# Kuntz-Lab/interactive-rate-tendons

Measured on AMD Instinct MI355X. Metric: FK+collision checks/sec (3-tendon, 256^3 voxel env), higher is better.
Workload: dtype f64

## Files before the change

interactive-rate-tendons_amd/csrc/sample_host.inc:

```
namespace {

int sample_box(tr_ctx *c, const double *lo, const double *hi, trk::SampleBox &box) {
  const int N = c->K.n_tendons, S = c->K.state_size;
  box = trk::SampleBox{};
  box.S = S;
  for (int d = 0; d < S; d++) {
    double a, b;
    if (lo && hi) { a = lo[d]; b = hi[d]; }
    else if (d < N) { a = 0.0; b = c->max_tension[(size_t)d]; }
    else if (c->K.enable_rotation && d == N) { a = -M_PI; b = M_PI; }
    else { a = 0.0; b = c->K.L; }
    if (!(b >= a) || !std::isfinite(a) || !std::isfinite(b)) return fail(c, TR_ERR_INVALID_ARG, "sampling bounds must be finite with hi >= lo");
    box.lo[d] = a; box.span[d] = b - a;
  }
  return TR_OK;
}

int ensure_sample_scratch(tr_ctx *c, int64_t batch, int64_t out_cap) {
  tr_ctx::Sampler &sm = c->samp;
  const size_t S = (size_t)c->K.state_size;
  int rc;
  if (!sm.d_ctr) {
    if ((rc = dev_alloc(c, &sm.d_ctr, 1))) return rc;
    HIP_TRY(c, hipHostMalloc((void **)&sm.h_ctr, sizeof(trk::SampleCounters), hipHostMallocDefault));
// ... 97 lines not shown
  return TR_OK;
}

}

extern "C" {

int tr_candidate_states_dev(tr_ctx *c, uint64_t seed, uint64_t first, int64_t count, const double *lo, const double *hi,
                            double *d_states, void *stream) {
  if (!c) return TR_ERR_INVALID_ARG;
  std::lock_guard<std::recursive_mutex> lock_(c->mu);
  if (count < 0 || (count > 0 && !d_states) || (!lo != !hi)) return fail(c, TR_ERR_INVALID_ARG, "bad argument");
  if (count == 0) return TR_OK;
  HIP_TRY(c, hipSetDevice(c->device));
  trk::SampleBox box;
  int rc;
  if ((rc = sample_box(c, lo, hi, box))) return rc;
  trk::launch_candidate_states(seed, first, count, box, d_states, (hipStream_t)stream);
  HIP_TRY(c, hipGetLastError());
  return TR_OK;
}

int tr_candidate_states(tr_ctx *c, uint64_t seed, uint64_t first, int64_t count, const double *lo, const double *hi, double *states) {
  if (!c) return TR_ERR_INVALID_ARG;
  std::lock_guard<std::recursive_mutex> lock_(c->mu);
  if (count < 0 || (count > 0 && !states) || (!lo != !hi)) return fail(c, TR_ERR_INVALID_ARG, "bad argument");
  if (count == 0) return TR_OK;
  HIP_TRY(c, hipSetDevice(c->device));
  int rc;
  const int S = c->K.state_size;
  const int64_t chunk = (int64_t)1 << 22;
  if ((rc = ensure_sample_scratch(c, std::min(count, chunk), c->samp.out_cap))) return rc;
  if ((rc = ensure_pipe(c))) return rc;
  hipStream_t s = c->pipe.s_comp;
  if ((rc = begin_dev_work(c, s))) return rc;
  trk::SampleBox box;
  if ((rc = sample_box(c, lo, hi, box))) return rc;
  for (int64_t off = 0; off < count; off += chunk) {
    const int64_t m = std::min(chunk, count - off);
    trk::launch_candidate_states(seed, first + (uint64_t)off, m, box, c->samp.states, s);
    HIP_TRY(c, hipGetLastError());
    HIP_TRY(c, hipMemcpyAsync(states + off * S, c->samp.states, (size_t)m * S * sizeof(double), hipMemcpyDeviceToHost, s));
    HIP_TRY(c, hipStreamSynchronize(s));
  }
  return note_dev_work(c, s);
}

static int validate_candidates_dev_impl(tr_ctx *c, uint64_t seed, uint64_t first, int64_t count, const double *lo, const double *hi,
                                        uint64_t *d_valid_bits, double *d_tips, uint8_t *d_flags, uint32_t *d_sig, void *stream) {
  if (!c) return TR_ERR_INVALID_ARG;
  std::lock_guard<std::recursive_mutex> lock_(c->mu);
  if (count < 0 || (count > 0 && !d_valid_bits) || (!lo != !hi)) return fail(c, TR_ERR_INVALID_ARG, "bad argument");
  if (count == 0) return TR_OK;
  if (first % 64) return fail(c, TR_ERR_INVALID_ARG, "first candidate must be a multiple of 64 (whole mask words)");
  HIP_TRY(c, hipSetDevice(c->device));
  hipStream_t s = (hipStream_t)stream;
  int rc;
  if ((rc = begin_dev_work(c, s))) return rc;
  trk::SampleBox box;
  if ((rc = sample_box(c, lo, hi, box))) return rc;
  const int S = c->K.state_size;
  const int64_t chunk = (int64_t)1 << 22;
  if ((rc = ensure_sample_scratch(c, std::min(count, chunk), c->samp.out_cap))) return rc;
  for (int64_t off = 0; off < count; off += chunk) {
    const int64_t m = std::min(chunk, count - off);
    trk::launch_candidate_states(seed, first + (uint64_t)off, m, box, c->samp.states, s);
    HIP_TRY(c, hipGetLastError());
// ... 97 lines not shown
  if (!c) return TR_ERR_INVALID_ARG;
  std::lock_guard<std::recursive_mutex> lock_(c->mu);
  if ((n_want > 0 && !d_states) || (!lo != !hi)) return fail(c, TR_ERR_INVALID_ARG, "bad argument");
  HIP_TRY(c, hipSetDevice(c->device));
  int rc;
  if ((rc = begin_dev_work(c, (hipStream_t)stream))) return rc;
  if ((rc = sample_valid_impl(c, seed, first_candidate, lo, hi, n_want, max_candidates, d_states, d_tips, d_index, n_accepted, n_tried,
                              (hipStream_t)stream))) return rc;
  return note_dev_work(c, (hipStream_t)stream);
}

int tr_sample_valid_vertices_sig_dev(tr_ctx *c, uint64_t seed, uint64_t first_candidate, const double *lo, const double *hi, int64_t n_want,
                                     int64_t max_candidates, double *d_states, double *d_tips, int64_t *d_index, uint32_t *d_sig,
                                     int64_t *n_accepted, int64_t *n_tried, void *stream) {
  if (!c) return TR_ERR_INVALID_ARG;
  std::lock_guard<std::recursive_mutex> lock_(c->mu);
  if ((n_want > 0 && (!d_states || !d_sig)) || (!lo != !hi)) return fail(c, TR_ERR_INVALID_ARG, "bad argument");
  HIP_TRY(c, hipSetDevice(c->device));
  int rc;
  if ((rc = begin_dev_work(c, (hipStream_t)stream))) return rc;
  if ((rc = sample_valid_impl(c, seed, first_candidate, lo, hi, n_want, max_candidates, d_states, d_tips, d_index, n_accepted, n_tried,
                              (hipStream_t)stream, d_sig))) return rc;
  return note_dev_work(c, (hipStream_t)stream);
}

int tr_sample_valid_vertices(tr_ctx *c, uint64_t seed, uint64_t first_candidate, const double *lo, const double *hi, int64_t n_want,
                             int64_t max_candidates, double *states, double *tips, int64_t *index, int64_t *n_accepted, int64_t *n_tried) {
  if (!c) return TR_ERR_INVALID_ARG;
  std::lock_guard<std::recursive_mutex> lock_(c->mu);
  if ((n_want > 0 && !states) || (!lo != !hi)) return fail(c, TR_ERR_INVALID_ARG, "bad argument");
  HIP_TRY(c, hipSetDevice(c->device));
  int rc;
  if ((rc = ensure_pipe(c))) return rc;
  hipStream_t s = c->pipe.s_comp;
  if ((rc = begin_dev_work(c, s))) return rc;
  int64_t have = 0;
  if ((rc = sample_valid_impl(c, seed, first_candidate, lo, hi, n_want, max_candidates, nullptr, nullptr, nullptr, &have, n_tried, s))) return rc;
  if (n_accepted) *n_accepted = have;
  if (have > 0) {
    const size_t S = (size_t)c->K.state_size;
    HIP_TRY(c, hipMemcpyAsync(states, c->samp.out_states, (size_t)have * S * sizeof(double), hipMemcpyDeviceToHost, s));
    if (tips) HIP_TRY(c, hipMemcpyAsync(tips, c->samp.out_tips, (size_t)have * 3 * sizeof(double), hipMemcpyDeviceToHost, s));
    if (index) HIP_TRY(c, hipMemcpyAsync(index, c->samp.out_index, (size_t)have * sizeof(int64_t), hipMemcpyDeviceToHost, s));
    HIP_TRY(c, hipStreamSynchronize(s));
  }
  return note_dev_work(c, s);
}

}
```

interactive-rate-tendons_amd/csrc/tendon_hip.hip:

```cpp
#include <hip/hip_runtime.h>
#include <sched.h>

#include <algorithm>
#include <cfloat>
#include <cmath>
#include <cstdio>
#include <cstdlib>
#include <cstring>
#include <functional>
#include <initializer_list>
#include <chrono>
#include <thread>
#include <ctime>
#include <limits>
#include <mutex>
#include <string>
#include <vector>

#include "../../include/tendon_hip.h"
#include "tr_types.hpp"
#include "fk_launch.hpp"
#include "fk_lin_launch.hpp"
#include "sweep_kernel.hpp"
#include "sphere_kernel.hpp"
#include "verdict_kernel.hpp"
#include "edge_kernel.hpp"
#include "edge_plan.hpp"
#include "routing_form.hpp"
#include "knn_kernel.hpp"
#include "cache_merge.hpp"
#include "env_kernel.hpp"
#include "sample.hpp"
#include "ik_kernel.hpp"
#include "fk_loaded_kernel.hpp"
#include "loaded_edge_kernel.hpp"
#include "loaded_roadmap_kernel.hpp"
#include "loaded_ik_kernel.hpp"
#include "loaded_sens_kernel.hpp"

void tr_dev_cache_trim();
struct tr_ctx;
namespace { void ik_release(tr_ctx *c); }
namespace { void shoot_release(tr_ctx *c); }
namespace { void ikl_release(tr_ctx *c); }

namespace {

std::string g_create_error;

struct Workspace {
  int64_t ld = 0;
  double *px = nullptr, *py = nullptr, *pz = nullptr, *acc = nullptr;
  double *Li = nullptr;
  double *homeLi = nullptr;
  int32_t *np = nullptr;
  uint8_t *conv = nullptr;
  int64_t st_cap = 0;
  double *states = nullptr;
  uint64_t *bits = nullptr;
  double *tips = nullptr;
  uint8_t *flags = nullptr;
// ... 106 lines not shown
  bool edge_lanes_fixed = false;
  bool edge_kernels_loaded = false;
  bool edge_queue = true;
  bool edge_queue_forced = false;
  int edge_queue_waves = 0;
  uint32_t edge_queue_last[4] = {0, 0, 0, 0};
  double edge_rate_seen = 0.0;
  bool edge_lane_guess_forced = false;
  double edge_lane_guess = 6.0;
  int64_t retract_sort_min = kRetractSortMin;
  bool rows_one_step = false;
  bool retract_wave_start = true;
  struct VerdictRing {
    static constexpr int kSlots = 16;
    trk::VerdictArgs *d_slots = nullptr, *h_slots = nullptr;
    hipEvent_t ev[kSlots];
    bool used[kSlots] = {};
    int next = 0;
  } vring;
  struct FusedRing {
    static constexpr int kSlots = 16;
    trk::FusedSweepArgs *d_slots = nullptr, *h_slots = nullptr;
    hipEvent_t ev[kSlots];
    bool used[kSlots] = {};
    int next = 0;
  } fused;
  struct KnnScratch { void *p[13] = {}; size_t cap[13] = {}; } knn;
  struct VoxStore { uint32_t *ids = nullptr; uint64_t *masks = nullptr; int64_t cap = 0, n = 0; } vstore;
  uint32_t *d_vids = nullptr; uint64_t *d_vmasks = nullptr; int32_t *d_vcounts = nullptr;
  uint64_t *d_vbits = nullptr;
  int64_t vox_cap = 0;
  int32_t *d_item_src = nullptr, *d_item_edge = nullptr; int64_t vox_items_cap = 0;
  struct Pipe {
    bool ready = false;
    int64_t chunk = 0;
    hipStream_t s_up = nullptr, s_comp = nullptr, s_down = nullptr;
    double *h_states[2] = {nullptr, nullptr}; double *h_tips[2] = {nullptr, nullptr};
    uint64_t *h_bits[2] = {nullptr, nullptr}; uint8_t *h_flags[2] = {nullptr, nullptr};
    hipEvent_t up[2], done[2], down[2];
  } pipe;
  hipEvent_t last_dev_ev = nullptr;
  bool last_dev_used = false;
  hipStream_t last_dev_stream = nullptr;
  struct Sampler {
    int64_t cap = 0;
    double *states = nullptr; uint64_t *bits = nullptr; double *tips = nullptr; uint32_t *wprefix = nullptr;
    uint32_t *wprefix2 = nullptr; int64_t wp2_cap = 0;
    trk::SampleCounters *d_ctr = nullptr, *h_ctr = nullptr;
    int64_t out_cap = 0;
    double *out_states = nullptr, *out_tips = nullptr; int64_t *out_index = nullptr;
    double rate_seen = 0.0;
    uint32_t *sig = nullptr; int64_t sig_cap = 0;
    int64_t *sig_index = nullptr; int64_t sig_index_cap = 0;
  } samp;
  void *h_stage = nullptr; size_t h_stage_cap = 0;
  struct IkDev {
    int64_t probs = 0, lanes = 0;
    double *xs = nullptr, *tips = nullptr;
    double *p = nullptr, *pn = nullptr, *f = nullptr, *J = nullptr, *des = nullptr;
    double *err2 = nullptr, *mu = nullptr, *nu = nullptr;
    int32_t *iters = nullptr, *calls = nullptr, *list[2] = {nullptr, nullptr};
    RoundCount count;
    double *io_s = nullptr, *io_3 = nullptr, *io_e = nullptr;
    int32_t *io_i = nullptr, *io_c = nullptr;
    DevOwner chunk, once;
  } ik;
  struct ShootDev {
    int64_t probs = 0, lanes = 0;
    double *xs = nullptr, *res = nullptr;
    double *p = nullptr, *pn = nullptr, *e = nullptr, *J = nullptr;
    double *err2 = nullptr, *mu = nullptr, *nu = nullptr;
    int32_t *iters = nullptr, *calls = nullptr, *list[2] = {nullptr, nullptr};
// ... 778 lines not shown
    }
  PolyK poly{};
  for (int j = 0; j < N; j++) {
    for (int i = 0; i < rb->n_a; i++) poly.C[j][i] = c->C[(size_t)j * rb->n_a + i];
    for (int i = 0; i < rb->n_m; i++) poly.D[j][i] = c->D[(size_t)j * rb->n_m + i];
    const int rdeg = poly_degree(&c->D[(size_t)j * rb->n_m], rb->n_m), tdeg = poly_degree(&c->C[(size_t)j * rb->n_a], rb->n_a);
    poly.home_kind[j] = (rdeg == 0 && tdeg == 0) ? 0 : ((rdeg == 0 && tdeg == 1) ? 1 : 2);
    const double d0 = poly.D[j][0], c1 = rb->n_a > 1 ? poly.C[j][1] : 0.0;
    poly.helix_scale[j] = std::sqrt(1 + d0 * d0 * c1 * c1);
  }

  auto bail = [&](const char *what) { std::string m = what; tr_destroy(c); return fail(nullptr, TR_ERR_HIP, m); };
  if (hipMalloc((void **)&c->d_poly, sizeof(PolyK)) != hipSuccess) return bail("hipMalloc(poly)");
  if (hipMemcpy(c->d_poly, &poly, sizeof(PolyK), hipMemcpyHostToDevice) != hipSuccess) return bail("hipMemcpy(poly)");
  if (hipMalloc((void **)&c->d_tgrid, c->t.size() * sizeof(double)) != hipSuccess ||
      hipMalloc((void **)&c->d_hl, hl.size() * sizeof(double)) != hipSuccess) return bail("hipMalloc(tgrid)");
  if (hipMemcpy(c->d_tgrid, c->t.data(), c->t.size() * sizeof(double), hipMemcpyHostToDevice) != hipSuccess ||
      hipMemcpy(c->d_hl, hl.data(), hl.size() * sizeof(double), hipMemcpyHostToDevice) != hipSuccess) return bail("hipMemcpy(tgrid)");
  if (hipMalloc((void **)&c->d_tab, tab.size() * sizeof(double)) != hipSuccess) return bail("hipMalloc(tab)");
  if (hipMemcpy(c->d_tab, tab.data(), tab.size() * sizeof(double), hipMemcpyHostToDevice) != hipSuccess) return bail("hipMemcpy(tab)");
  if (hipMalloc((void **)&c->d_steps, std::max<size_t>(1, c->steps.size()) * sizeof(StepK)) != hipSuccess) return bail("hipMalloc(steps)");
  if (!c->steps.empty() &&
      hipMemcpy(c->d_steps, c->steps.data(), c->steps.size() * sizeof(StepK), hipMemcpyHostToDevice) != hipSuccess) return bail("hipMemcpy(steps)");
  *out = c;
  return TR_OK;
}

void tr_destroy(tr_ctx *c) {
  if (!c) return;
  (void)hipSetDevice(c->device);
  (void)hipDeviceSynchronize();
  for (auto &v : c->events) for (auto &e : v) { (void)hipEventDestroy(e.a); (void)hipEventDestroy(e.b); }
  if (c->pipe.ready) {
    for (int b = 0; b < 2; b++) {
      (void)hipHostFree(c->pipe.h_states[b]); (void)hipHostFree(c->pipe.h_tips[b]); (void)hipHostFree(c->pipe.h_bits[b]); (void)hipHostFree(c->pipe.h_flags[b]);
      (void)hipEventDestroy(c->pipe.up[b]); (void)hipEventDestroy(c->pipe.done[b]); (void)hipEventDestroy(c->pipe.down[b]);
    }
    (void)hipStreamDestroy(c->pipe.s_up); (void)hipStreamDestroy(c->pipe.s_comp); (void)hipStreamDestroy(c->pipe.s_down);
  }
  Workspace &w = c->ws;
  void *ptrs[] = {c->d_tab, c->d_steps, c->d_poly, c->d_tgrid, c->d_hl, c->d_grid, c->d_near, w.homeLi, w.np, c->d_vids, c->d_vmasks, c->d_vcounts,
                  c->d_vbits, w.px, w.py, w.pz, w.acc, w.Li, w.conv,
                  w.states, w.bits, w.tips, w.flags, w.L, w.npts,
                  c->edge.lvl_states, c->edge.bits, c->edge.sample_edge, c->edge.sample_t, c->edge.open, c->edge.frontier,
                  c->edge.A, c->edge.B, c->edge.rel, c->edge.edge_ok, c->edge.nfk, c->edge.first_inv, c->edge.last_t, c->edge.nd, c->edge.cnt, c->edge.sig, c->edge.sig_np, c->edge.ix_states, c->edge.ix_idx, c->edge.open2, c->edge.lvl_states2, c->edge.q_remaining, c->edge.q_lvl_base, c->edge.q_lvl_cnt, c->edge.q_ctl, c->edge.q_args, c->d_envw[0], c->d_envw[1], c->d_sph_near, c->d_sph_tmp};
  for (void *p : ptrs) if (p) (void)hipFree(p);
  trk::merge_free(c->merge);
  if (c->fused.d_slots) { (void)hipFree(c->fused.d_slots); (void)hipHostFree(c->fused.h_slots); for (auto &e : c->fused.ev) (void)hipEventDestroy(e); }
  if (c->vring.d_slots) { (void)hipFree(c->vring.d_slots); (void)hipHostFree(c->vring.h_slots); for (auto &e : c->vring.ev) (void)hipEventDestroy(e); }
  if (c->last_dev_ev) (void)hipEventDestroy(c->last_dev_ev);
  {
    tr_ctx::Sampler &sm = c->samp;
    void *sp[] = {sm.states, sm.bits, sm.tips, sm.wprefix, sm.wprefix2, sm.d_ctr, sm.out_states, sm.out_tips, sm.out_index, sm.sig, sm.sig_index};
    for (void *q : sp) if (q) (void)hipFree(q);
    if (sm.h_ctr) (void)hipHostFree(sm.h_ctr);
  }
  if (c->d_item_src) (void)hipFree(c->d_item_src);
  if (c->d_item_edge) (void)hipFree(c->d_item_edge);
  for (void *q : c->knn.p) if (q) (void)hipFree(q);
  if (c->vstore.ids) (void)hipFree(c->vstore.ids);
  if (c->vstore.masks) (void)hipFree(c->vstore.masks);
  if (c->edge.q_hctl) (void)hipHostFree(c->edge.q_hctl);
  if (c->edge.q_hargs) (void)hipHostFree(c->edge.q_hargs);
  if (c->h_stage) (void)hipHostFree(c->h_stage);
  for (auto &ln : c->lane) {
    tr_ctx::RetractOrder &ro = ln.ro;
    void *lp[] = {ln.counters, ln.fb_list, ln.fb_count, ro.keys[0], ro.keys[1], ro.vals[0], ro.vals[1], ro.kbegin, ro.handoff};
    for (void *q : lp) if (q) (void)hipFree(q);
    if (ln.stream) (void)hipStreamDestroy(ln.stream);
    if (ln.hc) (void)hipHostFree(ln.hc);
    trk::merge_free(ro.ms);
// ... 349 lines not shown
  }
  (void)d_n_points;
  if ((rc = begin_dev_work(c, (hipStream_t)stream))) return rc;
  trk::SweepIn in{d_px, d_py, d_pz, nullptr, d_Li, d_converged, nullptr, c->ws.acc};
  if ((rc = launch_sweep(c, in, n, ld, check_voxels, d_valid_bits, d_flags, (hipStream_t)stream))) return rc;
  return note_dev_work(c, (hipStream_t)stream);
}

int tr_validate_shapes_retraction_dev(tr_ctx *c, int64_t n, int64_t ld, const double *d_px, const double *d_py,
                                      const double *d_pz, const int32_t *d_n_points, const double *d_Li,
                                      const double *d_home_Li, const uint8_t *d_converged, int check_voxels,
                                      uint64_t *d_valid_bits, uint8_t *d_flags, void *stream) {
  if (!c) return TR_ERR_INVALID_ARG;
  std::lock_guard<std::recursive_mutex> lock_(c->mu);
  if (!c->K.enable_retraction) return fail(c, TR_ERR_INVALID_ARG, "robot has no retraction: use tr_validate_shapes_dev");
  if (n < 0 || ld < n || (ld & 63)) return fail(c, TR_ERR_INVALID_ARG, "ld must be a multiple of 64 and >= n");
  if (n == 0) return TR_OK;
  if (!d_px || !d_py || !d_pz || !d_n_points || !d_Li || !d_home_Li || !d_converged || !d_valid_bits)
    return fail(c, TR_ERR_INVALID_ARG, "null device pointer");
  int rc;
  if (c->ws.ld < ld) {
    if (ld > c->max_chunk) return fail(c, TR_ERR_INVALID_ARG, "ld exceeds the workspace chunk size; call in smaller batches");
    if ((rc = ensure_workspace(c, ld))) return rc;
  }
  trk::SweepIn in{d_px, d_py, d_pz, d_n_points, d_Li, d_converged, d_home_Li, c->ws.acc};
  if ((rc = begin_dev_work(c, (hipStream_t)stream))) return rc;
  if ((rc = launch_sweep(c, in, n, ld, check_voxels, d_valid_bits, d_flags, (hipStream_t)stream))) return rc;
  return note_dev_work(c, (hipStream_t)stream);
}

}
namespace {
int validate_batch_dev_impl(tr_ctx *c, const double *d_states, int64_t n, uint64_t *d_valid_bits,
                            double *d_tips, uint8_t *d_flags, void *stream, uint32_t *d_sig = nullptr);
}
extern "C" {
int tr_validate_batch_dev(tr_ctx *c, const double *d_states, int64_t n, uint64_t *d_valid_bits,
                          double *d_tips, uint8_t *d_flags, void *stream) {
  if (!c) return TR_ERR_INVALID_ARG;
  std::lock_guard<std::recursive_mutex> lock_(c->mu);
  int rc;
  if ((rc = begin_dev_work(c, (hipStream_t)stream))) return rc;
  rc = validate_batch_dev_impl(c, d_states, n, d_valid_bits, d_tips, d_flags, stream);
  if (rc == TR_OK && n > 0) return note_dev_work(c, (hipStream_t)stream);
  return rc;
}
}
namespace {
int validate_batch_dev_impl(tr_ctx *c, const double *d_states, int64_t n, uint64_t *d_valid_bits,
                            double *d_tips, uint8_t *d_flags, void *stream, uint32_t *d_sig) {
  if (n < 0) return fail(c, TR_ERR_INVALID_ARG, "negative batch size");
  if (n == 0) return TR_OK;
  if (!d_states || !d_valid_bits) return fail(c, TR_ERR_INVALID_ARG, "null device pointer");
  if (!c->has_grid) return fail(c, TR_ERR_INVALID_ARG, "no obstacle grid set (tr_set_grid)");
  int rc;
  hipStream_t s = (hipStream_t)stream;
  const int S = c->K.state_size;
  const bool ret = c->K.enable_retraction;
  const int64_t sig_words = round_up(c->K.n_points, 16);
  if (d_sig && (c->fuse != 2 || ret || c->checker == TR_CHECKER_SPHERES)) return fail(c, TR_ERR_UNSUPPORTED, "signatures: backbone checker, no retraction, verdict-only schedule");
  if (c->fuse == 2) {
    const int64_t chunk = (int64_t)1 << 26;
    for (int64_t off = 0; off < n; off += chunk) {
      const int64_t m = std::min<int64_t>(chunk, n - off);
      if ((rc = launch_verdict(c, d_states + off * S, m, d_valid_bits + off / 64, d_tips ? d_tips + 3 * off : nullptr,
                               d_flags ? d_flags + off : nullptr, s, d_sig ? d_sig + off * sig_words : nullptr, d_sig ? sig_words : 0,
                               c->checker == TR_CHECKER_SPHERES))) return rc;
    }
    return TR_OK;
  }
  if ((rc = ensure_workspace(c, n))) return rc;
  Workspace &w = c->ws;
  for (int64_t off = 0; off < n; off += w.ld) {
    const int64_t m = std::min<int64_t>(w.ld, n - off);
    trk::FkOut out{w.px, w.py, w.pz, nullptr, nullptr, w.Li, d_tips ? d_tips + 3 * off : nullptr, w.conv,
                   ret ? w.np : nullptr, ret ? w.homeLi : nullptr};
    trk::SweepIn in{w.px, w.py, w.pz, ret ? w.np : nullptr, w.Li, w.conv, ret ? w.homeLi : nullptr, w.acc};
    if ((rc = launch_fk_sweep(c, d_states + off * S, m, w.ld, out, in, c->checker == TR_CHECKER_SPHERES ? 2 : 1, d_valid_bits + off / 64,
                              d_flags ? d_flags + off : nullptr, s))) return rc;
  }
  return TR_OK;
}
}
extern "C" {

namespace {
int ensure_pipe(tr_ctx *c) {
  tr_ctx::Pipe &p = c->pipe;
  if (p.ready) return TR_OK;
  int64_t CH = std::max<int64_t>(1 << 14, c->k1_round);
  if (const char *e = std::getenv("TENDON_HIP_PIPE_LOG2")) { const int v = std::atoi(e); if (v >= 12 && v <= 22) CH = (int64_t)1 << v; }
  const int S = c->K.state_size;
  HIP_TRY(c, hipStreamCreateWithFlags(&p.s_up, hipStreamNonBlocking));
  HIP_TRY(c, hipStreamCreateWithFlags(&p.s_comp, hipStreamNonBlocking));
  HIP_TRY(c, hipStreamCreateWithFlags(&p.s_down, hipStreamNonBlocking));
  for (int b = 0; b < 2; b++) {
    HIP_TRY(c, hipHostMalloc((void **)&p.h_states[b], (size_t)CH * S * sizeof(double), hipHostMallocDefault));
    HIP_TRY(c, hipHostMalloc((void **)&p.h_tips[b], (size_t)CH * 3 * sizeof(double), hipHostMallocDefault));
    HIP_TRY(c, hipHostMalloc((void **)&p.h_bits[b], (size_t)(CH / 64) * sizeof(uint64_t), hipHostMallocDefault));
    HIP_TRY(c, hipHostMalloc((void **)&p.h_flags[b], (size_t)CH, hipHostMallocDefault));
    HIP_TRY(c, hipEventCreateWithFlags(&p.up[b], hipEventDisableTiming));
    HIP_TRY(c, hipEventCreateWithFlags(&p.done[b], hipEventDisableTiming));
    HIP_TRY(c, hipEventCreateWithFlags(&p.down[b], hipEventDisableTiming));
  }
  p.chunk = CH;
  p.ready = true;
  return TR_OK;
}
}

int tr_validate_batch(tr_ctx *c, const double *states, int64_t n, uint64_t *valid_bits, double *tips, uint8_t *flags) {
  if (!c) return TR_ERR_INVALID_ARG;
  std::lock_guard<std::recursive_mutex> lock_(c->mu);
  if (n < 0 || (n > 0 && (!states || !valid_bits))) return fail(c, TR_ERR_INVALID_ARG, "bad argument");
  if (n == 0) return TR_OK;
  if (!c->has_grid) return fail(c, TR_ERR_INVALID_ARG, "no obstacle grid set (tr_set_grid)");
  HIP_TRY(c, hipSetDevice(c->device));
  int rc;
  if ((rc = ensure_pipe(c))) return rc;
  tr_ctx::Pipe &p = c->pipe;
  const int64_t CH = p.chunk;
  if (n <= kSmallBatch && n <= CH) {
    const int S = c->K.state_size;
    const bool verdict = c->fuse == 2;
    if ((rc = ensure_staging(c, n))) return rc;
    if (!verdict && (rc = ensure_workspace(c, n))) return rc;
    Workspace &w = c->ws;
    if ((rc = begin_dev_work(c, p.s_comp))) return rc;
    std::memcpy(p.h_states[0], states, (size_t)n * S * sizeof(double));
    HIP_TRY(c, hipMemcpyAsync(w.states, p.h_states[0], (size_t)n * S * sizeof(double), hipMemcpyHostToDevice, p.s_comp));
    if ((rc = validate_batch_dev_impl(c, w.states, n, w.bits, tips ? w.tips : nullptr, flags ? w.flags : nullptr, p.s_comp))) return rc;
    HIP_TRY(c, hipMemcpyAsync(p.h_bits[0], w.bits, (size_t)((n + 63) / 64) * sizeof(uint64_t), hipMemcpyDeviceToHost, p.s_comp));
    if (tips) HIP_TRY(c, hipMemcpyAsync(p.h_tips[0], w.tips, (size_t)n * 3 * sizeof(double), hipMemcpyDeviceToHost, p.s_comp));
    if (flags) HIP_TRY(c, hipMemcpyAsync(p.h_flags[0], w.flags, (size_t)n, hipMemcpyDeviceToHost, p.s_comp));
    HIP_TRY(c, hipStreamSynchronize(p.s_comp));
    c->last_dev_used = false;
    std::memcpy(valid_bits, p.h_bits[0], (size_t)((n + 63) / 64) * sizeof(uint64_t));
    if (tips) std::memcpy(tips, p.h_tips[0], (size_t)n * 3 * sizeof(double));
    if (flags) std::memcpy(flags, p.h_flags[0], (size_t)n);
    return TR_OK;
  }
  if ((rc = ensure_staging(c, std::min(n, 2 * CH)))) return rc;
  if (c->fuse != 2 && (rc = ensure_workspace(c, std::min(n, CH)))) return rc;
  HIP_TRY(c, hipDeviceSynchronize());
  Workspace &w = c->ws;
  const int S = c->K.state_size;
  const int64_t nchunks = (n + CH - 1) / CH;
  auto drain = [&](int64_t i) -> int {
    const int b = (int)(i & 1);
    const int64_t off = i * CH, m = std::min(CH, n - off);
    HIP_TRY(c, hipEventSynchronize(p.down[b]));
    std::memcpy(valid_bits + off / 64, p.h_bits[b], (size_t)((m + 63) / 64) * sizeof(uint64_t));
    if (tips) std::memcpy(tips + 3 * off, p.h_tips[b], (size_t)m * 3 * sizeof(double));
    if (flags) std::memcpy(flags + off, p.h_flags[b], (size_t)m);
    return TR_OK;
  };
  for (int64_t i = 0; i < nchunks; i++) {
    const int b = (int)(i & 1);
    const int64_t off = i * CH, m = std::min(CH, n - off);
    if (i >= 2 && (rc = drain(i - 2))) return rc;
    double *d_st = w.states + (size_t)b * CH * S;
    uint64_t *d_bits = w.bits + (size_t)b * (CH / 64);
    double *d_tips = w.tips + (size_t)b * CH * 3;
    uint8_t *d_flags = w.flags + (size_t)b * CH;
    std::memcpy(p.h_states[b], states + off * S, (size_t)m * S * sizeof(double));
    HIP_TRY(c, hipMemcpyAsync(d_st, p.h_states[b], (size_t)m * S * sizeof(double), hipMemcpyHostToDevice, p.s_up));
    HIP_TRY(c, hipEventRecord(p.up[b], p.s_up));
    HIP_TRY(c, hipStreamWaitEvent(p.s_comp, p.up[b], 0));
    if (i >= 2) HIP_TRY(c, hipStreamWaitEvent(p.s_comp, p.down[b], 0));
    if ((rc = validate_batch_dev_impl(c, d_st, m, d_bits, tips ? d_tips : nullptr, flags ? d_flags : nullptr, p.s_comp))) return rc;
    HIP_TRY(c, hipEventRecord(p.done[b], p.s_comp));
    HIP_TRY(c, hipStreamWaitEvent(p.s_down, p.done[b], 0));
    HIP_TRY(c, hipMemcpyAsync(p.h_bits[b], d_bits, (size_t)((m + 63) / 64) * sizeof(uint64_t), hipMemcpyDeviceToHost, p.s_down));
    if (tips) HIP_TRY(c, hipMemcpyAsync(p.h_tips[b], d_tips, (size_t)m * 3 * sizeof(double), hipMemcpyDeviceToHost, p.s_down));
    if (flags) HIP_TRY(c, hipMemcpyAsync(p.h_flags[b], d_flags, (size_t)m, hipMemcpyDeviceToHost, p.s_down));
    HIP_TRY(c, hipEventRecord(p.down[b], p.s_down));
  }
  for (int64_t i = std::max<int64_t>(0, nchunks - 2); i < nchunks; i++)
    if ((rc = drain(i))) return rc;
  return TR_OK;
}

int tr_check_cached_dev(tr_ctx *c, const uint32_t *d_ids, const uint64_t *d_masks, const int64_t *d_offsets,
                        int64_t n_items, uint64_t *d_hit_bits, void *stream) {
  if (!c) return TR_ERR_INVALID_ARG;
  std::lock_guard<std::recursive_mutex> lock_(c->mu);
  if (n_items < 0) return fail(c, TR_ERR_INVALID_ARG, "negative item count");
  if (n_items == 0) return TR_OK;
  if (!c->has_grid) return fail(c, TR_ERR_INVALID_ARG, "no obstacle grid set (tr_set_grid)");
  if (!d_ids || !d_masks || !d_offsets || !d_hit_bits) return fail(c, TR_ERR_INVALID_ARG, "null device pointer");
  hipStream_t s = (hipStream_t)stream;
  ProfScope ps(c, 2, s);
  const unsigned grid = (unsigned)((n_items + 3) / 4);
  HIP_TRY(c, hipMemsetAsync(d_hit_bits, 0, (size_t)((n_items + 63) / 64) * sizeof(uint64_t), s));
  hipLaunchKernelGGL(trk::cached_blocks_vs_grid, dim3(grid), dim3(64), 0, s, d_ids, d_masks, d_offsets, n_items,
                     c->d_grid, c->n_blocks, d_hit_bits);
  HIP_TRY(c, hipGetLastError());
  return TR_OK;
}

int tr_check_cached_subset_dev(tr_ctx *c, const uint32_t *d_ids, const uint64_t *d_masks, const int64_t *d_offsets,
                               int64_t n_items, const int32_t *d_list, int64_t n_list, uint8_t *d_hit, void *stream) {
  if (!c) return TR_ERR_INVALID_ARG;
  std::lock_guard<std::recursive_mutex> lock_(c->mu);
  if (n_items < 0 || n_list < 0) return fail(c, TR_ERR_INVALID_ARG, "negative count");
  if (n_list == 0) return TR_OK;
  if (!c->has_grid) return fail(c, TR_ERR_INVALID_ARG, "no obstacle grid set (tr_set_grid)");
  if (!d_ids || !d_masks || !d_offsets || !d_list || !d_hit) return fail(c, TR_ERR_INVALID_ARG, "null device pointer");
  hipStream_t s = (hipStream_t)stream;
  ProfScope ps(c, 2, s);
  hipLaunchKernelGGL(trk::cached_subset_vs_grid, dim3((unsigned)((n_list + 15) / 16)), dim3(256), 0, s, d_ids, d_masks, d_offsets,
                     d_list, n_list, n_items, c->d_grid, c->n_blocks, d_hit);
// ... 485 lines not shown
```

profiles/probe_host_pipe.py:

```python
#!/usr/bin/env python3
import importlib
import json
import os
import sys
import time

import numpy as np

ROOT = os.path.dirname(os.path.dirname(os.path.abspath(__file__)))
sys.path.insert(0, ROOT)


def main():
    import torch
    irt = importlib.import_module("interactive-rate-tendons_amd")
    W = irt.workloads
    robot = W.robot_config2()
    vox, _ = W.reach_environment(seed=7, n_spheres=64)
    n = 1 << 20
    states = W.random_states(robot, n, seed=3, tau_max=10.0)
    out = {}
    for log2 in (None, 14, 15, 16, 17, 18):
        if log2 is None:
            os.environ.pop("TENDON_HIP_PIPE_LOG2", None)
        else:
            os.environ["TENDON_HIP_PIPE_LOG2"] = str(log2)
        chk = irt.VoxelBackboneValidityChecker(robot, irt.VoxelEnvironment(), vox)
        eng = chk.engine
        for _ in range(2):
            eng.validate_batch(states)
        ts = []
        for _ in range(8):
            t0 = time.perf_counter()
            eng.validate_batch(states)
            ts.append(time.perf_counter() - t0)
        ts2 = []
        for _ in range(8):
            t0 = time.perf_counter()
            eng.validate_batch(states, want_tips=False, want_flags=False)
            ts2.append(time.perf_counter() - t0)
        d = torch.from_numpy(states).cuda()
        bits = torch.zeros(n // 64, dtype=torch.int64, device="cuda")
        tips = torch.zeros(n, 3, dtype=torch.float64, device="cuda")
        eng.validate_batch_dev(d, n, bits, tips)
        torch.cuda.synchronize()
        t0 = time.perf_counter()
# ... 17 lines not shown
```

Before: 137.6 million.

## Grade host pipeline chunk sizes and alternate compute across two lanes

Measured after the change: 137.8 million, median of 6. About the same (+0.1%).

```diff
diff --git a/interactive-rate-tendons_amd/csrc/pipe_schedule.hpp b/interactive-rate-tendons_amd/csrc/pipe_schedule.hpp
--- /dev/null
+++ b/interactive-rate-tendons_amd/csrc/pipe_schedule.hpp
@@ -0,0 +1,55 @@
+#pragma once
+#include <algorithm>
+#include <cstdint>
+#include <vector>
+
+namespace pipe_schedule {
+
+struct Chunk { int64_t offset, count; };
+
+constexpr int64_t kWave = 64;
+constexpr int64_t kGrade = 2;
+
+inline int64_t end_size(int64_t steady) {
+  const int64_t q = steady / kGrade / kWave * kWave;
+  return std::min(steady, std::max(q, kWave));
+}
+
+inline int64_t max_chunks(int64_t n, int64_t steady) {
+  int64_t ramp = 0;
+  for (int64_t s = end_size(steady); s < steady; s *= 2) ramp++;
+  return n / steady + 2 * ramp + 2;
+}
+inline std::vector<Chunk> graded(int64_t n, int64_t steady) {
+  std::vector<Chunk> out;
+  if (n <= 0 || steady < kWave) return out;
+  steady = steady / kWave * kWave;
+  const int64_t q = end_size(steady);
+  std::vector<int64_t> up, down;
+  for (int64_t s = q; s < steady; s *= 2) up.push_back(s);
+  down.assign(up.rbegin(), up.rend());
+  int64_t ramps = 0;
+  for (int64_t s : up) ramps += 2 * s;
+  std::vector<int64_t> counts;
+  if (n < ramps + steady) {
+    const int64_t k = (n + steady - 1) / steady;
+    const int64_t each = std::min(steady, ((n + k - 1) / k + kWave - 1) / kWave * kWave);
+    for (int64_t left = n; left > 0; left -= each) counts.push_back(std::min(each, left));
+  } else {
+    counts = up;
+    int64_t mid = n - ramps;
+    for (; mid >= steady; mid -= steady) counts.push_back(steady);
+    const int64_t odd = mid % kWave;
+    if (mid - odd > 0) counts.push_back(mid - odd);
+    counts.insert(counts.end(), down.begin(), down.end());
+    if (odd > 0) {
+      if (!down.empty() && counts.back() + odd <= steady) counts.back() += odd;
+      else counts.push_back(odd);
+    }
+  }
+  int64_t off = 0;
+  for (int64_t m : counts) { out.push_back(Chunk{off, m}); off += m; }
+  return out;
+}
+
+}
diff --git a/interactive-rate-tendons_amd/csrc/sample_host.inc b/interactive-rate-tendons_amd/csrc/sample_host.inc
--- a/interactive-rate-tendons_amd/csrc/sample_host.inc
+++ b/interactive-rate-tendons_amd/csrc/sample_host.inc
@@ -153,7 +153,7 @@
   const int64_t chunk = (int64_t)1 << 22;
   if ((rc = ensure_sample_scratch(c, std::min(count, chunk), c->samp.out_cap))) return rc;
   if ((rc = ensure_pipe(c))) return rc;
-  hipStream_t s = c->pipe.s_comp;
+  hipStream_t s = c->pipe.s_comp[0];
   if ((rc = begin_dev_work(c, s))) return rc;
   trk::SampleBox box;
   if ((rc = sample_box(c, lo, hi, box))) return rc;
@@ -317,7 +317,7 @@
   HIP_TRY(c, hipSetDevice(c->device));
   int rc;
   if ((rc = ensure_pipe(c))) return rc;
-  hipStream_t s = c->pipe.s_comp;
+  hipStream_t s = c->pipe.s_comp[0];
   if ((rc = begin_dev_work(c, s))) return rc;
   int64_t have = 0;
   if ((rc = sample_valid_impl(c, seed, first_candidate, lo, hi, n_want, max_candidates, nullptr, nullptr, nullptr, &have, n_tried, s))) return rc;
diff --git a/interactive-rate-tendons_amd/csrc/tendon_hip.hip b/interactive-rate-tendons_amd/csrc/tendon_hip.hip
--- a/interactive-rate-tendons_amd/csrc/tendon_hip.hip
+++ b/interactive-rate-tendons_amd/csrc/tendon_hip.hip
@@ -27,6 +27,7 @@
 #include "edge_kernel.hpp"
 #include "edge_plan.hpp"
 #include "routing_form.hpp"
+#include "pipe_schedule.hpp"
 #include "knn_kernel.hpp"
 #include "cache_merge.hpp"
 #include "env_kernel.hpp"
@@ -199,12 +200,13 @@
   int64_t vox_cap = 0;
   int32_t *d_item_src = nullptr, *d_item_edge = nullptr; int64_t vox_items_cap = 0;
   struct Pipe {
+    static constexpr int kSlots = 2;
     bool ready = false;
     int64_t chunk = 0;
-    hipStream_t s_up = nullptr, s_comp = nullptr, s_down = nullptr;
-    double *h_states[2] = {nullptr, nullptr}; double *h_tips[2] = {nullptr, nullptr};
-    uint64_t *h_bits[2] = {nullptr, nullptr}; uint8_t *h_flags[2] = {nullptr, nullptr};
-    hipEvent_t up[2], done[2], down[2];
+    hipStream_t s_up = nullptr, s_comp[2] = {nullptr, nullptr};
+    double *h_states[kSlots] = {}; double *h_tips[kSlots] = {};
+    uint64_t *h_bits[kSlots] = {}; uint8_t *h_flags[kSlots] = {};
+    hipEvent_t up[kSlots], done[kSlots], down[kSlots];
   } pipe;
   hipEvent_t last_dev_ev = nullptr;
   bool last_dev_used = false;
@@ -1049,11 +1051,11 @@
   (void)hipDeviceSynchronize();
   for (auto &v : c->events) for (auto &e : v) { (void)hipEventDestroy(e.a); (void)hipEventDestroy(e.b); }
   if (c->pipe.ready) {
-    for (int b = 0; b < 2; b++) {
+    for (int b = 0; b < tr_ctx::Pipe::kSlots; b++) {
       (void)hipHostFree(c->pipe.h_states[b]); (void)hipHostFree(c->pipe.h_tips[b]); (void)hipHostFree(c->pipe.h_bits[b]); (void)hipHostFree(c->pipe.h_flags[b]);
       (void)hipEventDestroy(c->pipe.up[b]); (void)hipEventDestroy(c->pipe.done[b]); (void)hipEventDestroy(c->pipe.down[b]);
     }
-    (void)hipStreamDestroy(c->pipe.s_up); (void)hipStreamDestroy(c->pipe.s_comp); (void)hipStreamDestroy(c->pipe.s_down);
+    (void)hipStreamDestroy(c->pipe.s_up); for (hipStream_t s : c->pipe.s_comp) (void)hipStreamDestroy(s);
   }
   Workspace &w = c->ws;
   void *ptrs[] = {c->d_tab, c->d_steps, c->d_poly, c->d_tgrid, c->d_hl, c->d_grid, c->d_near, w.homeLi, w.np, c->d_vids, c->d_vmasks, c->d_vcounts,
@@ -1469,7 +1471,7 @@
 }
 namespace {
 int validate_batch_dev_impl(tr_ctx *c, const double *d_states, int64_t n, uint64_t *d_valid_bits,
-                            double *d_tips, uint8_t *d_flags, void *stream, uint32_t *d_sig = nullptr);
+                            double *d_tips, uint8_t *d_flags, void *stream, uint32_t *d_sig = nullptr, int lane = 0);
 }
 extern "C" {
 int tr_validate_batch_dev(tr_ctx *c, const double *d_states, int64_t n, uint64_t *d_valid_bits,
@@ -1485,7 +1487,7 @@
 }
 namespace {
 int validate_batch_dev_impl(tr_ctx *c, const double *d_states, int64_t n, uint64_t *d_valid_bits,
-                            double *d_tips, uint8_t *d_flags, void *stream, uint32_t *d_sig) {
+                            double *d_tips, uint8_t *d_flags, void *stream, uint32_t *d_sig, int lane) {
   if (n < 0) return fail(c, TR_ERR_INVALID_ARG, "negative batch size");
   if (n == 0) return TR_OK;
   if (!d_states || !d_valid_bits) return fail(c, TR_ERR_INVALID_ARG, "null device pointer");
@@ -1502,7 +1504,7 @@
       const int64_t m = std::min<int64_t>(chunk, n - off);
       if ((rc = launch_verdict(c, d_states + off * S, m, d_valid_bits + off / 64, d_tips ? d_tips + 3 * off : nullptr,
                                d_flags ? d_flags + off : nullptr, s, d_sig ? d_sig + off * sig_words : nullptr, d_sig ? sig_words : 0,
-                               c->checker == TR_CHECKER_SPHERES))) return rc;
+                               c->checker == TR_CHECKER_SPHERES, nullptr, lane))) return rc;
     }
     return TR_OK;
   }
@@ -1522,6 +1524,62 @@
 extern "C" {
 
 namespace {
+#ifdef TRK_PIPE_TIMELINE
+struct PipeTimeline {
+  enum { UP0, UP1, K0, K1, DN1, NEV };
+  struct Chunk { int64_t m = 0; int lane = 0; hipEvent_t ev[NEV] = {}; double in0 = 0, in1 = 0, out0 = 0, out1 = 0, wait0 = 0; };
+  std::vector<Chunk> ch;
+  hipEvent_t base = nullptr;
+  std::chrono::steady_clock::time_point t_entry, t_base;
+  static double ms(std::chrono::steady_clock::time_point a, std::chrono::steady_clock::time_point b) { return std::chrono::duration<double, std::milli>(b - a).count(); }
+  double now() const { return ms(t_base, std::chrono::steady_clock::now()); }
+  void enter() { t_entry = std::chrono::steady_clock::now(); }
+  void start(size_t nchunks, hipStream_t s) {
+    ch.assign(nchunks, Chunk{});
+    (void)hipEventCreate(&base);
+    (void)hipEventRecord(base, s);
+    t_base = std::chrono::steady_clock::now();
+  }
+  void mark(int64_t i, int which, hipStream_t s) { (void)hipEventCreate(&ch[(size_t)i].ev[which]); (void)hipEventRecord(ch[(size_t)i].ev[which], s); }
+  void report(int64_t n) {
+    const double t_end = now();
+    (void)hipDeviceSynchronize();
+    auto at = [&](hipEvent_t e) { float t = 0; (void)hipEventElapsedTime(&t, base, e); return (double)t; };
+    std::fprintf(stderr, "pipe_timeline n %lld chunks %zu  (ms after the entry synchronisation; host clock for in/out, device events for up/kern/down)\n", (long long)n, ch.size());
+    std::fprintf(stderr, "pipe_timeline # chunk lane count | stage-in | upload | kernels | download-end | wait-begin copy-out\n");
+    std::vector<std::pair<double, double>> iv;
+    double in_sum = 0, out_sum = 0, wait_sum = 0;
+    for (size_t i = 0; i < ch.size(); i++) {
+      Chunk &q = ch[i];
+      const double u0 = at(q.ev[UP0]), u1 = at(q.ev[UP1]), k0 = at(q.ev[K0]), k1 = at(q.ev[K1]), d1 = at(q.ev[DN1]);
+      iv.push_back({k0, k1});
+      in_sum += q.in1 - q.in0; out_sum += q.out1 - q.out0; wait_sum += q.out0 - q.wait0;
+      std::fprintf(stderr, "pipe_timeline %2zu %d %7lld | %7.3f %7.3f | %7.3f %7.3f | %7.3f %7.3f | %7.3f | %7.3f %7.3f %7.3f\n", i, q.lane, (long long)q.m,
+                   q.in0, q.in1, u0, u1, k0, k1, d1, q.wait0, q.out0, q.out1);
+      for (hipEvent_t e : q.ev) (void)hipEventDestroy(e);
+    }
+    std::sort(iv.begin(), iv.end());
+    double busy = 0, first = iv.front().first, last = 0, cur0 = iv.front().first, cur1 = iv.front().second;
+    for (auto &v : iv) {
+      last = std::max(last, v.second);
+      if (v.first > cur1) { busy += cur1 - cur0; cur0 = v.first; cur1 = v.second; } else cur1 = std::max(cur1, v.second);
+    }
+    busy += cur1 - cur0;
+    std::fprintf(stderr, "pipe_timeline span_ms %.3f (entry to the synchronisation's return %.3f, from there to the call's end %.3f)\n",
+                 ms(t_entry, t_base) + t_end, ms(t_entry, t_base), t_end);
+    std::fprintf(stderr, "pipe_timeline busy_in_kernels_ms %.3f\n", busy);
+    std::fprintf(stderr, "pipe_timeline idle_before_first_kernel_ms %.3f (+ %.3f before the synchronisation returned)\n", first, ms(t_entry, t_base));
+    std::fprintf(stderr, "pipe_timeline idle_after_last_kernel_ms %.3f\n", t_end - last);
+    std::fprintf(stderr, "pipe_timeline gaps_between_chunk_kernels_ms %.3f\n", (last - first) - busy);
+    std::fprintf(stderr, "pipe_timeline host_stage_in_ms %.3f host_copy_out_ms %.3f host_waiting_for_downloads_ms %.3f\n", in_sum, out_sum, wait_sum);
+    (void)hipEventDestroy(base);
+  }
+};
+#define PIPE_TL(x) x
+#else
+#define PIPE_TL(x)
+#endif
+
 int ensure_pipe(tr_ctx *c) {
   tr_ctx::Pipe &p = c->pipe;
   if (p.ready) return TR_OK;
@@ -1529,9 +1587,8 @@
   if (const char *e = std::getenv("TENDON_HIP_PIPE_LOG2")) { const int v = std::atoi(e); if (v >= 12 && v <= 22) CH = (int64_t)1 << v; }
   const int S = c->K.state_size;
   HIP_TRY(c, hipStreamCreateWithFlags(&p.s_up, hipStreamNonBlocking));
-  HIP_TRY(c, hipStreamCreateWithFlags(&p.s_comp, hipStreamNonBlocking));
-  HIP_TRY(c, hipStreamCreateWithFlags(&p.s_down, hipStreamNonBlocking));
-  for (int b = 0; b < 2; b++) {
+  for (hipStream_t &s : p.s_comp) HIP_TRY(c, hipStreamCreateWithFlags(&s, hipStreamNonBlocking));
+  for (int b = 0; b < tr_ctx::Pipe::kSlots; b++) {
     HIP_TRY(c, hipHostMalloc((void **)&p.h_states[b], (size_t)CH * S * sizeof(double), hipHostMallocDefault));
     HIP_TRY(c, hipHostMalloc((void **)&p.h_tips[b], (size_t)CH * 3 * sizeof(double), hipHostMallocDefault));
     HIP_TRY(c, hipHostMalloc((void **)&p.h_bits[b], (size_t)(CH / 64) * sizeof(uint64_t), hipHostMallocDefault));
@@ -1554,6 +1611,7 @@
   if (!c->has_grid) return fail(c, TR_ERR_INVALID_ARG, "no obstacle grid set (tr_set_grid)");
   HIP_TRY(c, hipSetDevice(c->device));
   int rc;
+  PIPE_TL(PipeTimeline tl; tl.enter());
   if ((rc = ensure_pipe(c))) return rc;
   tr_ctx::Pipe &p = c->pipe;
   const int64_t CH = p.chunk;
@@ -1563,58 +1621,86 @@
     if ((rc = ensure_staging(c, n))) return rc;
     if (!verdict && (rc = ensure_workspace(c, n))) return rc;
     Workspace &w = c->ws;
-    if ((rc = begin_dev_work(c, p.s_comp))) return rc;
+    if ((rc = begin_dev_work(c, p.s_comp[0]))) return rc;
     std::memcpy(p.h_states[0], states, (size_t)n * S * sizeof(double));
-    HIP_TRY(c, hipMemcpyAsync(w.states, p.h_states[0], (size_t)n * S * sizeof(double), hipMemcpyHostToDevice, p.s_comp));
-    if ((rc = validate_batch_dev_impl(c, w.states, n, w.bits, tips ? w.tips : nullptr, flags ? w.flags : nullptr, p.s_comp))) return rc;
-    HIP_TRY(c, hipMemcpyAsync(p.h_bits[0], w.bits, (size_t)((n + 63) / 64) * sizeof(uint64_t), hipMemcpyDeviceToHost, p.s_comp));
-    if (tips) HIP_TRY(c, hipMemcpyAsync(p.h_tips[0], w.tips, (size_t)n * 3 * sizeof(double), hipMemcpyDeviceToHost, p.s_comp));
-    if (flags) HIP_TRY(c, hipMemcpyAsync(p.h_flags[0], w.flags, (size_t)n, hipMemcpyDeviceToHost, p.s_comp));
-    HIP_TRY(c, hipStreamSynchronize(p.s_comp));
+    HIP_TRY(c, hipMemcpyAsync(w.states, p.h_states[0], (size_t)n * S * sizeof(double), hipMemcpyHostToDevice, p.s_comp[0]));
+    if ((rc = validate_batch_dev_impl(c, w.states, n, w.bits, tips ? w.tips : nullptr, flags ? w.flags : nullptr, p.s_comp[0]))) return rc;
+    HIP_TRY(c, hipMemcpyAsync(p.h_bits[0], w.bits, (size_t)((n + 63) / 64) * sizeof(uint64_t), hipMemcpyDeviceToHost, p.s_comp[0]));
+    if (tips) HIP_TRY(c, hipMemcpyAsync(p.h_tips[0], w.tips, (size_t)n * 3 * sizeof(double), hipMemcpyDeviceToHost, p.s_comp[0]));
+    if (flags) HIP_TRY(c, hipMemcpyAsync(p.h_flags[0], w.flags, (size_t)n, hipMemcpyDeviceToHost, p.s_comp[0]));
+    HIP_TRY(c, hipStreamSynchronize(p.s_comp[0]));
     c->last_dev_used = false;
     std::memcpy(valid_bits, p.h_bits[0], (size_t)((n + 63) / 64) * sizeof(uint64_t));
     if (tips) std::memcpy(tips, p.h_tips[0], (size_t)n * 3 * sizeof(double));
     if (flags) std::memcpy(flags, p.h_flags[0], (size_t)n);
     return TR_OK;
   }
-  if ((rc = ensure_staging(c, std::min(n, 2 * CH)))) return rc;
+  const std::vector<pipe_schedule::Chunk> sched = pipe_schedule::graded(n, CH);
+  const int64_t nchunks = (int64_t)sched.size();
+  constexpr int NS = tr_ctx::Pipe::kSlots;
+  if ((rc = ensure_staging(c, nchunks > 1 ? std::min<int64_t>(nchunks, NS) * CH : n))) return rc;
   if (c->fuse != 2 && (rc = ensure_workspace(c, std::min(n, CH)))) return rc;
+  const bool lanes = c->fuse == 2 && nchunks > 1 && 2 * c->fb_cap <= c->max_chunk;
+  if (lanes) {
+    const int64_t most = round_up(std::min(n, CH), 64);
+    for (int l = 0; l < 2; l++) {
+      if ((rc = ensure_lane_fallback(c, l, most))) return rc;
+      if (c->K.enable_retraction && c->retract_sort_min > 0 && most >= c->retract_sort_min && (rc = ensure_lane_order(c, l, most))) return rc;
+    }
+    if ((rc = ensure_workspace(c, 2 * c->fb_cap))) return rc;
+  }
   HIP_TRY(c, hipDeviceSynchronize());
+  c->last_dev_used = false;
   Workspace &w = c->ws;
   const int S = c->K.state_size;
-  const int64_t nchunks = (n + CH - 1) / CH;
+  PIPE_TL(tl.start((size_t)nchunks, p.s_comp[0]));
   auto drain = [&](int64_t i) -> int {
-    const int b = (int)(i & 1);
-    const int64_t off = i * CH, m = std::min(CH, n - off);
+    const int b = (int)(i % NS);
+    const int64_t off = sched[(size_t)i].offset, m = sched[(size_t)i].count;
+    PIPE_TL(tl.ch[(size_t)i].wait0 = tl.now());
     HIP_TRY(c, hipEventSynchronize(p.down[b]));
+    PIPE_TL(tl.ch[(size_t)i].out0 = tl.now());
     std::memcpy(valid_bits + off / 64, p.h_bits[b], (size_t)((m + 63) / 64) * sizeof(uint64_t));
     if (tips) std::memcpy(tips + 3 * off, p.h_tips[b], (size_t)m * 3 * sizeof(double));
     if (flags) std::memcpy(flags + off, p.h_flags[b], (size_t)m);
+    PIPE_TL(tl.ch[(size_t)i].out1 = tl.now());
     return TR_OK;
   };
   for (int64_t i = 0; i < nchunks; i++) {
-    const int b = (int)(i & 1);
-    const int64_t off = i * CH, m = std::min(CH, n - off);
-    if (i >= 2 && (rc = drain(i - 2))) return rc;
+    const int b = (int)(i % NS), lane = lanes ? (int)(i & 1) : 0;
+    const bool reused = i >= NS;
+    const hipStream_t sc = p.s_comp[lane], sd = lanes ? sc : p.s_comp[1];
+    const int64_t off = sched[(size_t)i].offset, m = sched[(size_t)i].count;
     double *d_st = w.states + (size_t)b * CH * S;
     uint64_t *d_bits = w.bits + (size_t)b * (CH / 64);
     double *d_tips = w.tips + (size_t)b * CH * 3;
     uint8_t *d_flags = w.flags + (size_t)b * CH;
+    if (reused) HIP_TRY(c, hipEventSynchronize(p.up[b]));
+    PIPE_TL(tl.ch[(size_t)i].m = m; tl.ch[(size_t)i].lane = lane; tl.ch[(size_t)i].in0 = tl.now());
     std::memcpy(p.h_states[b], states + off * S, (size_t)m * S * sizeof(double));
+    PIPE_TL(tl.ch[(size_t)i].in1 = tl.now());
+    if (reused) HIP_TRY(c, hipStreamWaitEvent(p.s_up, p.done[b], 0));
+    PIPE_TL(tl.mark(i, PipeTimeline::UP0, p.s_up));
     HIP_TRY(c, hipMemcpyAsync(d_st, p.h_states[b], (size_t)m * S * sizeof(double), hipMemcpyHostToDevice, p.s_up));
+    PIPE_TL(tl.mark(i, PipeTimeline::UP1, p.s_up));
     HIP_TRY(c, hipEventRecord(p.up[b], p.s_up));
-    HIP_TRY(c, hipStreamWaitEvent(p.s_comp, p.up[b], 0));
-    if (i >= 2) HIP_TRY(c, hipStreamWaitEvent(p.s_comp, p.down[b], 0));
-    if ((rc = validate_batch_dev_impl(c, d_st, m, d_bits, tips ? d_tips : nullptr, flags ? d_flags : nullptr, p.s_comp))) return rc;
-    HIP_TRY(c, hipEventRecord(p.done[b], p.s_comp));
-    HIP_TRY(c, hipStreamWaitEvent(p.s_down, p.done[b], 0));
-    HIP_TRY(c, hipMemcpyAsync(p.h_bits[b], d_bits, (size_t)((m + 63) / 64) * sizeof(uint64_t), hipMemcpyDeviceToHost, p.s_down));
-    if (tips) HIP_TRY(c, hipMemcpyAsync(p.h_tips[b], d_tips, (size_t)m * 3 * sizeof(double), hipMemcpyDeviceToHost, p.s_down));
-    if (flags) HIP_TRY(c, hipMemcpyAsync(p.h_flags[b], d_flags, (size_t)m, hipMemcpyDeviceToHost, p.s_down));
-    HIP_TRY(c, hipEventRecord(p.down[b], p.s_down));
-  }
-  for (int64_t i = std::max<int64_t>(0, nchunks - 2); i < nchunks; i++)
+    HIP_TRY(c, hipStreamWaitEvent(sc, p.up[b], 0));
+    if (reused) HIP_TRY(c, hipStreamWaitEvent(sc, p.down[b], 0));
+    PIPE_TL(tl.mark(i, PipeTimeline::K0, sc));
+    if ((rc = validate_batch_dev_impl(c, d_st, m, d_bits, tips ? d_tips : nullptr, flags ? d_flags : nullptr, sc, nullptr, lane))) return rc;
+    PIPE_TL(tl.mark(i, PipeTimeline::K1, sc));
+    HIP_TRY(c, hipEventRecord(p.done[b], sc));
+    if (reused && (rc = drain(i - NS))) return rc;
+    HIP_TRY(c, hipStreamWaitEvent(sd, p.done[b], 0));
+    HIP_TRY(c, hipMemcpyAsync(p.h_bits[b], d_bits, (size_t)((m + 63) / 64) * sizeof(uint64_t), hipMemcpyDeviceToHost, sd));
+    if (tips) HIP_TRY(c, hipMemcpyAsync(p.h_tips[b], d_tips, (size_t)m * 3 * sizeof(double), hipMemcpyDeviceToHost, sd));
+    if (flags) HIP_TRY(c, hipMemcpyAsync(p.h_flags[b], d_flags, (size_t)m, hipMemcpyDeviceToHost, sd));
+    PIPE_TL(tl.mark(i, PipeTimeline::DN1, sd));
+    HIP_TRY(c, hipEventRecord(p.down[b], sd));
+  }
+  for (int64_t i = std::max<int64_t>(0, nchunks - NS); i < nchunks; i++)
     if ((rc = drain(i))) return rc;
+  PIPE_TL(tl.report(n));
   return TR_OK;
 }
 
diff --git a/profiles/probe_host_pipe.py b/profiles/probe_host_pipe.py
--- a/profiles/probe_host_pipe.py
+++ b/profiles/probe_host_pipe.py
@@ -11,7 +11,91 @@
 sys.path.insert(0, ROOT)
 
 
+N_LOG2 = 20
+
+
+def _setup():
+    irt = importlib.import_module("interactive-rate-tendons_amd")
+    W = irt.workloads
+    robot = W.robot_config2()
+    vox, _ = W.reach_environment(seed=7, n_spheres=64)
+    chk = irt.VoxelBackboneValidityChecker(robot, irt.VoxelEnvironment(), vox)
+    n = 1 << N_LOG2
+    states = irt.distributed.candidate_states(robot, seed=2024, start=0, count=n, tau_max=10.0)
+    return irt, chk, states
+
+
+def timeline():
+    _, chk, states = _setup()
+    for k in range(3):
+        print("pipe_timeline_call %d" % k, file=sys.stderr, flush=True)
+        chk.engine.validate_batch(states)
+
+
+def ab(label, out):
+    import torch
+    irt, chk, states = _setup()
+    eng, n = chk.engine, len(states)
+    for _ in range(2):
+        eng.validate_batch(states, True, False)
+    ts = []
+    for _ in range(7):
+        t0 = time.perf_counter()
+        eng.validate_batch(states, True, False)
+        ts.append(1e3 * (time.perf_counter() - t0))
+    d = torch.from_numpy(states).cuda()
+    bits = torch.zeros(n // 64, dtype=torch.int64, device="cuda")
+    tips = torch.zeros(n, 3, dtype=torch.float64, device="cuda")
+    for _ in range(3):
+        eng.validate_batch_dev(d, n, bits, tips)
+    torch.cuda.synchronize()
+    t0 = time.perf_counter()
+    for _ in range(20):
+        eng.validate_batch_dev(d, n, bits, tips)
+    torch.cuda.synchronize()
+    rec = {"label": label, "n_log2": N_LOG2, "lib": os.environ.get("TENDON_HIP_LIB"), "host_ms_median": float(np.median(ts)), "host_ms": ts,
+           "ms_per_step": 1e3 * (time.perf_counter() - t0) / 20}
+    print(json.dumps(rec), flush=True)
+    with open(out, "a") as f:
+        f.write(json.dumps(rec) + "\n")
+
+
+def ab_summary(src, out):
+    recs = [json.loads(l) for l in open(src) if l.strip()]
+    par = [r for r in recs if r["label"] == "parent"]
+    br = [r for r in recs if r["label"] == "branch"]
+    pairs = list(zip(par, br))
+    gains = [p["host_ms_median"] - b["host_ms_median"] for p, b in pairs]
+    spread = max(p["host_ms_median"] for p in par) - min(p["host_ms_median"] for p in par)
+    overhead = [p["host_ms_median"] - p["ms_per_step"] for p in par]
+    res = {"runs": recs, "parent_medians_ms": [p["host_ms_median"] for p in par], "branch_medians_ms": [b["host_ms_median"] for b in br],
+           "gains_ms": gains, "mean_gain_ms": float(np.mean(gains)), "parent_spread_ms": spread,
+           "branch_faster_in_every_pair": all(g > 0 for g in gains), "mean_gain_at_least_3x_parent_spread": float(np.mean(gains)) >= 3 * spread,
+           "parent_overhead_ms": float(np.mean(overhead)), "gain_share_of_parent_overhead": float(np.mean(gains) / np.mean(overhead)),
+           "checks_per_s_parent": (1 << 20) / (1e-3 * float(np.mean([p["host_ms_median"] for p in par]))),
+           "checks_per_s_branch": (1 << 20) / (1e-3 * float(np.mean([b["host_ms_median"] for b in br])))}
+    with open(out, "w") as f:
+        json.dump(res, f, indent=1)
+    print(json.dumps({k: v for k, v in res.items() if k != "runs"}, indent=1))
+
+
 def main():
+    import argparse
+    ap = argparse.ArgumentParser()
+    ap.add_argument("--timeline", action="store_true")
+    ap.add_argument("--ab")
+    ap.add_argument("--ab-summary")
+    ap.add_argument("--out")
+    ap.add_argument("--n-log2", type=int, default=20, help="batch size of --timeline and --ab (default: the headline's 2^20)")
+    args = ap.parse_args()
+    global N_LOG2
+    N_LOG2 = args.n_log2
+    if args.timeline:
+        return timeline()
+    if args.ab:
+        return ab(args.ab, args.out)
+    if args.ab_summary:
+        return ab_summary(args.ab_summary, args.out)
     import torch
     irt = importlib.import_module("interactive-rate-tendons_amd")
     W = irt.workloads
```
